# menonsamir/spiral

Measured on AMD Instinct MI355X. Metric: server ms/query + DB GB/s vs HBM roofline, 2^20 x 256B, lower is better.
Workload: dtype u32 residues, 32x32->64-bit integer MAC (two 28-bit CRT primes)

## Files before the change

spiral_amd/csrc/kernels.h:

```cpp
#pragma once
#include <hip/hip_runtime.h>
#include <stdint.h>
#include <stdlib.h>
#include "common.h"

namespace spiral {

struct IndexMap {
    uint32_t inner, outer_stride, off;
    __host__ __device__ uint32_t operator()(uint32_t b) const { return (b / inner) * outer_stride + (b % inner) + off; }
};
inline IndexMap identity_map() { return IndexMap{1u, 1u, 0u}; }

#ifdef SPIRAL_TUNING
inline const char* tuning_env(const char* name) { return getenv(name); }
#else
inline const char* tuning_env(const char*) { return nullptr; }
#endif
struct Options {
    int fold_pair = 1, fold_chain = 1, fwd2 = -1;
    uint32_t fold_blocks = 768, sweep_mfma_min = 2, fwd2_min = 8192;
    size_t db_stage_bytes = (size_t)64 << 20;
    int one_image = 1;
    uint32_t pack_item_group = 0;
};
Options& options();

#ifndef SPIRAL_MAX_LANES
#define SPIRAL_MAX_LANES 8
#endif
constexpr uint32_t kMaxLanes = SPIRAL_MAX_LANES;
struct Lanes {
    uint32_t n = 1;
    int64_t off[kMaxLanes] = {};
#ifdef __HIPCC__
    __device__ __forceinline__ int64_t here() const {
        const uint32_t z = blockIdx.z;
        int64_t o = 0;
#pragma unroll
        for (uint32_t q = 1; q < kMaxLanes; q++) o = z == q ? off[q] : o;
        return o;
    }
    __device__ __forceinline__ int64_t at(int64_t stride) const { return (int64_t)blockIdx.z * stride; }
#endif
};
#ifdef __HIPCC__
template <class T>
__device__ __forceinline__ void lane_shift(T*& p, int64_t words) {
    if (p) p = reinterpret_cast<T*>(reinterpret_cast<uintptr_t>(p) + (intptr_t)words * 8);
}
#endif
struct NoLanes {
    uint32_t n = 1;
#ifdef __HIPCC__
    __device__ __forceinline__ int64_t here() const { return 0; }
    __device__ __forceinline__ int64_t at(int64_t) const { return 0; }
#endif
};
struct Slots {
    uint32_t n = 1;
    int64_t stride = 0;
#ifdef __HIPCC__
    __device__ __forceinline__ int64_t here() const { return (int64_t)blockIdx.z * stride; }
    __device__ __forceinline__ int64_t at(int64_t s) const { return (int64_t)blockIdx.z * s; }
#endif
};
template <class P>
inline typename P::NoLanesT no_lanes(const P& p) {
    typename P::NoLanesT q{};
    static_cast<typename P::Core&>(q) = static_cast<const typename P::Core&>(p);
    return q;
}

struct DeviceTables {
    uint4* fwd = nullptr;
    uint4* inv = nullptr;
    uint64_t* neg1 = nullptr;
    uint64_t* neg1s = nullptr;
};
int tables_get(int device, DeviceTables* out);
void tables_host_rows(uint64_t* out8x2048);

constexpr bool lazy_ok(uint32_t terms) { return (unsigned __int128)terms * (2ull * kP - 1ull) * (kP - 1ull) < ((unsigned __int128)1 << 64); }
static_assert(lazy_ok(56) && lazy_ok(2 * 56) && lazy_ok(128) && !lazy_ok(129), "u64 accumulators hold up to 128 lazy products");

enum FwdLoad : uint32_t {
    LD_RAW = 0,
    LD_DIGIT = 1,
    LD_SDIGIT = 2,
    LD_LIMBS = 3,
    LD_DBGEN = 4,
    LD_PDIGIT = 6,
    LD_DBGEN1 = 7,
    LD_SDIFF = 8,
    LD_PDIFF = 9,
    LD_EXPAND = 5,
    LD_WIRE = 10,
};
constexpr uint32_t kWireCoeffBytes = 7;
constexpr uint32_t kWirePolyBytes = kWireCoeffBytes * 2048u;
enum FwdStore : uint32_t {
    ST_PK = 0,
    ST_REF = 1,
    ST_DB = 2,
    ST_DB1 = 3,
};
enum PackMap : uint32_t {
    PM_GSW = 0,
    PM_FOLD = 1,
    PM_PACK = 2,
};
struct FwdParamsCore {
    const uint64_t* src;
    uint64_t* dst;
    IndexMap src_map;
    IndexMap dst_map;
    uint32_t n_digits;
    uint32_t inv_n_digits, inv_te, inv_to;
    uint32_t bits;
    uint32_t ell;
    uint32_t tinv;
    uint32_t lazy_out;
    uint32_t fold_np;
    uint32_t pmode, pk_num_per;
    uint32_t trial;
    uint64_t total_n;
    uint32_t cnt_e, t_e, t_o;
    const uint8_t* items;
    uint32_t coeff_bits;
    uint64_t items_first;
    uint32_t* err;
    uint64_t seed, p_db;
    uint64_t item_base;
    uint32_t num_per, dim0_shard, j0;
};
template <class L>
struct FwdParamsT : FwdParamsCore {
    using Core = FwdParamsCore;
    using NoLanesT = FwdParamsT<NoLanes>;
    L lanes;
};
using FwdParams = FwdParamsT<Lanes>;
void launch_ntt_forward(const DeviceTables& t, const FwdParams& p, uint32_t load, uint32_t store, uint32_t nblocks, hipStream_t s);

struct ExpandActive {
    uint32_t e_off, o_stride_m1, o_off;
    __host__ __device__ uint32_t index(uint32_t a, uint32_t cnt_e) const {
        return a < cnt_e ? 2u * (a + e_off) : 2u * ((a - cnt_e) * (o_stride_m1 + 1u) + o_off) + 1u;
    }
};

enum InvStore : uint32_t {
    IST_CRT = 0,
    IST_LIMBS = 1,
};
struct InvParamsCore {
    const uint64_t* src;
    uint64_t* dst;
    IndexMap src_map, dst_map;
    uint32_t pre_reduce;
    uint32_t src_ref;
    uint32_t split;
    IndexMap src_map2;
    uint64_t* cv;
    const uint64_t* neg1;
    const uint64_t* neg1s;
    uint32_t num_in, cnt_e;
    ExpandActive act;
    uint32_t auto_t;
    uint32_t create_here;
    const uint64_t* query;
};
template <class L>
struct InvParamsT : InvParamsCore {
    using Core = InvParamsCore;
    using NoLanesT = InvParamsT<NoLanes>;
    L lanes;
// ... 200 lines not shown
```

spiral_amd/csrc/server.cpp:

```cpp
#include <atomic>

#include "db_image.h"
#include "message.h"

using namespace spiral;

thread_local std::string spiral::host::g_err;
using namespace spiral::host;

static std::atomic<uint64_t> g_captures{0};

spiral::Options& spiral::options() {
    static Options o = [] {
        Options v;
        if (const char* e = getenv("SPIRAL_FOLD_PAIR")) v.fold_pair = atoi(e) != 0;
        if (const char* e = getenv("SPIRAL_SWEEP_MFMA")) v.sweep_mfma_min = (uint32_t)strtoul(e, nullptr, 10);
        if (const char* e = getenv("SPIRAL_DB_STAGE_BYTES")) v.db_stage_bytes = (size_t)strtoull(e, nullptr, 10);
        return v;
    }();
    return o;
}

enum GraphId : int {
    G_PRE = 0,
// ... 187 lines not shown

int srv_join_side(spiral_gpu_server* S) {
    if (S->side_pending) {
        HIP_OK(hipStreamWaitEvent(S->stream, S->ev_join, 0));
        S->side_pending = false;
    }
    return 0;
}

enum LaneNeeds : uint32_t {
    NEED_QUERY = 1,
    NEED_DB = 2,
    NEED_RECORDS = 4,
    SHARDED = 8,
    NO_CAPTURE = 16,
    SWEEP_ONLY = 32,
    SHARD_LANES = SHARDED | NO_CAPTURE,
};

int check_lanes(spiral_gpu_server* const* servers, uint32_t n, const char* what, uint32_t needs, Lanes* lanes) {
    if (!servers || n == 0) return fail("%s: no servers", what);
    if (n > kMaxLanes) return fail("%s: at most %u clients per batch", what, kMaxLanes);
    for (uint32_t b = 0; b < n; b++)
        if (!servers[b]) return fail("%s: null server %u", what, b);
    spiral_gpu_server* S = servers[0];
    HIP_OK(hipSetDevice(S->device));
    const bool whole = !(needs & SWEEP_ONLY), sharded = needs & SHARDED;
    lanes->n = n;
    for (uint32_t b = 0; b < n; b++) {
        spiral_gpu_server* L = servers[b];
        if (whole && (((needs & NEED_QUERY) && !L->have_query) || !L->have_pp)) return fail("%s: server %u needs its query and public parameters set first", what, b);
        if ((needs & NEED_DB) && !L->img->loaded) return fail("%s: server %u has no database", what, b);
        if ((needs & NEED_RECORDS) && !L->have_records) return fail("%s: server %u has not converted its query (run_pre first)", what, b);
        if (L->device != S->device || L->dim0_shard != S->dim0_shard || L->s.num_per != S->s.num_per ||
            (whole && (memcmp(&L->p, &S->p, sizeof(S->p)) != 0 || L->j0 != S->j0 || L->j1 != S->j1 || L->cv.words != S->cv.words)))
            return fail("%s: server %u differs from server 0 in parameters, device or shard", what, b);
        if (L->img != S->img) return fail("%s: server %u does not sweep server 0's database image (create_lane / share_db)", what, b);
        if ((sharded || !whole) && L->fold_g_log != S->fold_g_log)
            return fail("%s: server %u has %u fold ranks, server 0 has %u", what, b, 1u << L->fold_g_log, 1u << S->fold_g_log);
        if (sharded && (L->ex_shard.g_log != S->ex_shard.g_log || L->ex_shard.rank != S->ex_shard.rank))
            return fail("%s: server %u has another expansion shard than server 0", what, b);
        if (whole && !sharded && (L->acc != L->acc_own.p || L->fold_g_log || L->ex_shard.g_log))
            return fail("%s: server %u has an external accumulator, fold ranks or a sharded expansion set", what, b);
        if (L->sweep_k_log || (whole && (L->keep_cts || L->overlap || L->side_pending || L->fold_pair != S->fold_pair || L->fold_chain != S->fold_chain)))
            return fail("%s: server %u has keep_cts, a split or staged schedule or other fold options set", what, b);
        for (uint32_t c = 0; c < b; c++)
            if (servers[c] == L) return fail("%s: server %u listed twice", what, b);
        hipStreamCaptureStatus cs = hipStreamCaptureStatusNone;
        if (needs & NO_CAPTURE) HIP_OK(hipStreamIsCapturing(L->stream, &cs));
        if (cs != hipStreamCaptureStatusNone) return fail("%s: server %u's stream is capturing (call it outside stream capture)", what, b);
        lanes->off[b] = L->w_left.p - S->w_left.p;
    }
    return 0;
}

int lanes_join(spiral_gpu_server* const* servers, uint32_t n) {
    spiral_gpu_server* S = servers[0];
    for (uint32_t b = 1; b < n; b++) {
        if (servers[b]->stream == S->stream) continue;
        HIP_OK(hipEventRecord(servers[b]->ev_batch, servers[b]->stream));
        HIP_OK(hipStreamWaitEvent(S->stream, servers[b]->ev_batch, 0));
    }
    return 0;
}
int lanes_release(spiral_gpu_server* const* servers, uint32_t n) {
    spiral_gpu_server* S = servers[0];
    bool other = false;
    for (uint32_t b = 1; b < n; b++) other |= servers[b]->stream != S->stream;
    if (other) HIP_OK(hipEventRecord(S->ev_batch, S->stream));
    for (uint32_t b = 1; b < n; b++)
        if (servers[b]->stream != S->stream) HIP_OK(hipStreamWaitEvent(servers[b]->stream, S->ev_batch, 0));
    return 0;
}

void mark_raw_stale(spiral_gpu_server* const* servers, uint32_t n) {
    for (uint32_t b = 0; b < n; b++) servers[b]->raw_from_acc = false;
}
void mark_swept(spiral_gpu_server* const* servers, uint32_t n) {
    for (uint32_t b = 0; b < n; b++) servers[b]->have_records = true;
    mark_raw_stale(servers, n);
}

void server_records(spiral_gpu_server* const* servers, uint32_t n, const uint32_t** qs, uint64_t** acc) {
    for (uint32_t b = 0; b < n; b++) {
        qs[b] = (const uint32_t*)servers[b]->qs.p;
        acc[b] = servers[b]->acc;
    }
}

int take_pub_params(spiral_gpu_server* S, Form form, const MessageIn& in, const char* what) {
    if (!S) return fail("null server");
    HIP_OK(hipSetDevice(S->device));
    const MessageLayout m = pub_params_layout(S->p, S->s);
    if (form == FORM_NTT && check_ntt_parts(m, in, what)) return -1;
    uint64_t* const dst[kMessageParts] = {S->w_left.p, S->w_right.p, S->w.p, S->v.p};
    S->have_pp = false;
    if (ingest(form, IngestOn{S->stage, S->wire_in, S->tb, S->stream}, m, dst, in, what)) return -1;
    S->have_pp = true;
    return 0;
}
int take_query(spiral_gpu_server* S, Form form, const MessageIn& in, const char* what) {
    if (!S) return fail("null server");
    HIP_OK(hipSetDevice(S->device));
    const MessageLayout m = query_layout(S->p, S->s);
    if (form == FORM_NTT && check_ntt_parts(m, in, what)) return -1;
    uint64_t* const dst[kMessageParts] = {S->query.p};
    S->have_query = S->have_records = false;
    if (ingest(form, IngestOn{S->stage, S->wire_in, S->tb, S->stream}, m, dst, in, what)) return -1;
    S->have_query = true;
    return 0;
}
size_t base_message_bytes(const spiral_gpu_params* p, MessageLayout (*layout)(const spiral_gpu_params&, const spiral_gpu_shape&), Form form) {
    spiral_gpu_shape s;
    return shape_of(p, &s) ? 0 : message_bytes(layout(*p, s), form);
}

int download_pk_as_ref(spiral_gpu_server* S, const uint64_t* pk, IndexMap map, uint64_t* host, size_t npolys) {
    if (npolys == 0) return 0;
    const size_t chunk = 4096;
    if (S->stage.words < std::min(npolys, chunk) * kRefNtt) {
        S->stage.release();
        if (S->stage.alloc(std::min(npolys, chunk) * kRefNtt)) return -1;
    }
    for (size_t done = 0; done < npolys; done += chunk) {
        const size_t n = std::min(chunk, npolys - done);
        IndexMap m = map;
        m.off += (uint32_t)(done / map.inner) * map.outer_stride;
        launch_pk_to_ref(pk, S->stage.p, (uint32_t)n, m, S->stream);
        HIP_OK(hipMemcpyAsync(host + done * kRefNtt, S->stage.p, n * kRefNtt * sizeof(uint64_t), hipMemcpyDeviceToHost, S->stream));
        HIP_OK(hipStreamSynchronize(S->stream));
    }
    return 0;
}

}

extern "C" {

int spiral_gpu_abi_version(void) { return SPIRAL_GPU_ABI_VERSION; }

int spiral_gpu_set_option(const char* name, int64_t value) {
    if (!name) return fail("null option name");
    Options& o = options();
    const std::string n = name;
    if (n == "fold_pair") o.fold_pair = value != 0;
    else if (n == "fold_chain") o.fold_chain = value != 0;
    else if (n == "fold_blocks" && value >= 0) o.fold_blocks = (uint32_t)value;
    else if (n == "sweep_mfma_min" && value >= 0) o.sweep_mfma_min = (uint32_t)value;
    else if (n == "one_image") o.one_image = value != 0;
    else if (n == "fwd2" && value >= -1 && value <= 1) o.fwd2 = (int)value;
    else if (n == "fwd2_min" && value >= 0) o.fwd2_min = (uint32_t)value;
    else if (n == "db_stage_bytes" && value > 0) o.db_stage_bytes = (size_t)value;
    else if (n == "pack_item_group" && value >= 0 && value <= 0xFFFFFFFFll) o.pack_item_group = (uint32_t)value;
    else return fail("unknown option '%s' or value %lld out of range", name, (long long)value);
    return 0;
}
int spiral_gpu_get_option(const char* name, int64_t* value) {
    if (!name || !value) return fail("null argument");
    const Options& o = options();
    const std::string n = name;
    if (n == "fold_pair") *value = o.fold_pair;
    else if (n == "fold_chain") *value = o.fold_chain;
    else if (n == "fold_blocks") *value = o.fold_blocks;
    else if (n == "sweep_mfma_min") *value = o.sweep_mfma_min;
    else if (n == "one_image") *value = o.one_image;
    else if (n == "fwd2") *value = o.fwd2;
    else if (n == "fwd2_min") *value = o.fwd2_min;
    else if (n == "db_stage_bytes") *value = (int64_t)o.db_stage_bytes;
    else if (n == "pack_item_group") *value = o.pack_item_group;
    else if (n == "graph_captures") *value = (int64_t)g_captures.load();
    else return fail("unknown option '%s'", name);
    return 0;
}
const char* spiral_gpu_last_error(void) { return g_err.c_str(); }
int spiral_gpu_device_count(void) {
    int n = 0;
    if (hipGetDeviceCount(&n) != hipSuccess) return 0;
    return n;
}
int spiral_gpu_get_shape(const spiral_gpu_params* p, spiral_gpu_shape* out) { return shape_of(p, out); }
int spiral_gpu_get_tables(uint64_t* out) {
    if (!out) return fail("null argument");
    tables_host_rows(out);
    return 0;
}

int spiral_gpu_ntt_forward(uint64_t* operand, size_t npolys) {
    DeviceTables tb;
    if (current_tables(&tb)) return -1;
    Scratch sc;
    uint64_t* d = sc.upload(operand, npolys * kRefNtt);
    if (!d) return fail("device allocation/upload failed");
    FwdParams fp{};
    fp.src = d;
    fp.dst = d;
    fp.src_map = fp.dst_map = identity_map();
    fp.n_digits = 1;
    launch_ntt_forward(tb, fp, LD_LIMBS, ST_REF, (uint32_t)npolys, 0);
    HIP_OK(hipMemcpy(operand, d, npolys * kRefNtt * sizeof(uint64_t), hipMemcpyDeviceToHost));
    return 0;
}

int spiral_gpu_ntt_inverse(uint64_t* operand, size_t npolys) {
    DeviceTables tb;
    if (current_tables(&tb)) return -1;
    Scratch sc;
    uint64_t* d = sc.upload(operand, npolys * kRefNtt);
    if (!d) return fail("device allocation/upload failed");
    InvParams ip{};
    ip.src = d;
    ip.dst = d;
    ip.src_map = ip.dst_map = identity_map();
    ip.src_ref = 1;
    ip.pre_reduce = 1;
    launch_ntt_inverse(tb, ip, IST_LIMBS, (uint32_t)npolys, 0);
    HIP_OK(hipMemcpy(operand, d, npolys * kRefNtt * sizeof(uint64_t), hipMemcpyDeviceToHost));
    return 0;
}

int spiral_gpu_to_ntt(uint64_t* out, const uint64_t* in, size_t npolys, int reduce) {
    DeviceTables tb;
    if (current_tables(&tb)) return -1;
    Scratch sc;
    uint64_t* d_in = sc.upload(in, npolys * kN);
    uint64_t* d_out = sc.get(npolys * kRefNtt);
    if (!d_in || !d_out) return fail("device allocation/upload failed");
    FwdParams fp{};
    fp.src = d_in;
    fp.dst = d_out;
    fp.src_map = fp.dst_map = identity_map();
    fp.n_digits = 1;
    if (reduce) {
        launch_ntt_forward(tb, fp, LD_RAW, ST_REF, (uint32_t)npolys, 0);
    } else {
        uint64_t* d_pk = sc.get(npolys * kN);
        if (!d_pk) return fail("device allocation failed");
        fp.dst = d_pk;
        fp.bits = 32;
        launch_ntt_forward(tb, fp, LD_DIGIT, ST_PK, (uint32_t)npolys, 0);
        launch_pk_to_ref(d_pk, d_out, (uint32_t)npolys, identity_map(), 0);
    }
    HIP_OK(hipMemcpy(out, d_out, npolys * kRefNtt * sizeof(uint64_t), hipMemcpyDeviceToHost));
    return 0;
}

int spiral_gpu_from_ntt(uint64_t* out, const uint64_t* in, size_t npolys) {
    DeviceTables tb;
    if (current_tables(&tb)) return -1;
    Scratch sc;
    uint64_t* d_in = sc.upload(in, npolys * kRefNtt);
    uint64_t* d_out = sc.get(npolys * kN);
    if (!d_in || !d_out) return fail("device allocation/upload failed");
    InvParams ip{};
    ip.src = d_in;
    ip.dst = d_out;
    ip.src_map = ip.dst_map = identity_map();
    ip.src_ref = 1;
    ip.pre_reduce = 1;
    launch_ntt_inverse(tb, ip, IST_CRT, (uint32_t)npolys, 0);
    HIP_OK(hipMemcpy(out, d_out, npolys * kN * sizeof(uint64_t), hipMemcpyDeviceToHost));
    return 0;
}


int spiral_gpu_time_ntt(size_t npolys, int iters, float* fwd_ms, float* inv_ms) {
    if (!fwd_ms || !inv_ms || iters <= 0 || npolys == 0) return fail("bad argument");
    DeviceTables tb;
    if (current_tables(&tb)) return -1;
    Scratch sc;
    uint64_t* d_raw = sc.get(npolys * kN);
    uint64_t* d_pk = sc.get(npolys * kN);
    if (!d_raw || !d_pk) return fail("device allocation failed");
    HIP_OK(hipMemset(d_raw, 0x5a, npolys * kN * sizeof(uint64_t)));
    hipEvent_t e[3];
    for (auto& x : e) HIP_OK(hipEventCreate(&x));
    FwdParams fp{};
    fp.src = d_raw;
    fp.dst = d_pk;
    fp.src_map = fp.dst_map = identity_map();
    fp.n_digits = 1;
    InvParams ip{};
    ip.src = d_pk;
    ip.dst = d_raw;
    ip.src_map = ip.dst_map = identity_map();
    launch_ntt_forward(tb, fp, LD_RAW, ST_PK, (uint32_t)npolys, 0);
    launch_ntt_inverse(tb, ip, IST_CRT, (uint32_t)npolys, 0);
    HIP_OK(hipEventRecord(e[0], 0));
    for (int i = 0; i < iters; i++) launch_ntt_forward(tb, fp, LD_RAW, ST_PK, (uint32_t)npolys, 0);
    HIP_OK(hipEventRecord(e[1], 0));
    for (int i = 0; i < iters; i++) launch_ntt_inverse(tb, ip, IST_CRT, (uint32_t)npolys, 0);
    HIP_OK(hipEventRecord(e[2], 0));
    HIP_OK(hipEventSynchronize(e[2]));
    HIP_OK(hipEventElapsedTime(fwd_ms, e[0], e[1]));
    HIP_OK(hipEventElapsedTime(inv_ms, e[1], e[2]));
    *fwd_ms /= iters;
    *inv_ms /= iters;
    for (auto& x : e) (void)hipEventDestroy(x);
    return 0;
}

int spiral_gpu_time_ntt_digits(size_t npolys, uint32_t n_digits, int iters, float* ms) {
    if (!ms || iters <= 0 || npolys == 0 || n_digits < 1 || n_digits > 56) return fail("bad argument");
    DeviceTables tb;
    if (current_tables(&tb)) return -1;
    Scratch sc;
    uint64_t* d_raw = sc.get(npolys * kN);
    uint64_t* d_pk = sc.get(npolys * n_digits * kN);
    if (!d_raw || !d_pk) return fail("device allocation failed");
    HIP_OK(hipMemset(d_raw, 0x5a, npolys * kN * sizeof(uint64_t)));
    hipEvent_t e[2];
    for (auto& x : e) HIP_OK(hipEventCreate(&x));
    FwdParams fp{};
    fp.src = d_raw;
    fp.dst = d_pk;
    fp.src_map = fp.dst_map = identity_map();
    fp.n_digits = n_digits;
    fp.bits = get_bits_per(n_digits);
    launch_ntt_forward(tb, fp, LD_DIGIT, ST_PK, (uint32_t)(npolys * n_digits), 0);
    HIP_OK(hipEventRecord(e[0], 0));
    for (int i = 0; i < iters; i++) launch_ntt_forward(tb, fp, LD_DIGIT, ST_PK, (uint32_t)(npolys * n_digits), 0);
    HIP_OK(hipEventRecord(e[1], 0));
    HIP_OK(hipEventSynchronize(e[1]));
// ... 1774 lines not shown
```

spiral_amd/csrc/sweep.hip:

```cpp
#include <cstdlib>
#include "common.h"
#include "kernels.h"

namespace spiral {

typedef unsigned long long u64x2 __attribute__((ext_vector_type(2)));

__device__ __forceinline__ void mac6(uint64_t (&a)[6], uint32_t p0, uint32_t p1, uint32_t p2, uint32_t b0, uint32_t b1, uint32_t b2, uint64_t w) {
    const uint32_t bl = lo32(w), bh = hi32(w);
    a[0] += (uint64_t)p0 * bl;
    a[1] += (uint64_t)p1 * bl;
    a[2] += (uint64_t)p2 * bl;
    a[3] += (uint64_t)b0 * bh;
    a[4] += (uint64_t)b1 * bh;
    a[5] += (uint64_t)b2 * bh;
}
__device__ __forceinline__ void mac_j(uint64_t (&a)[6], const uint4* q, uint64_t w0, uint64_t w1) {
    const uint4 qa = q[0], qb = q[1], qc = q[2];
    mac6(a, qa.x, qa.y, qa.z, qa.w, qb.x, qb.y, w0);
    mac6(a, qb.z, qb.w, qc.x, qc.y, qc.z, qc.w, w1);
}
__device__ __forceinline__ void reduce6(uint64_t (&a)[6]) {
#pragma unroll
    for (int r = 0; r < 3; r++) {
        a[r] = mod_p(a[r]);
        a[3 + r] = mod_b(a[3 + r]);
    }
}
__device__ __forceinline__ void store_acc(uint64_t* acc, const uint64_t (&a)[6], uint32_t ic, uint32_t z, uint32_t g_log, uint32_t ls_log) {
    const uint32_t i0 = ic >> 1, c = ic & 1u;
    const uint32_t ii = acc_pos(i0, g_log, ls_log);
#pragma unroll
    for (uint32_t r = 0; r < 3; r++) acc[((size_t)(6u * ii + 2u * r + c)) * kN + z] = pack((uint32_t)a[r], (uint32_t)a[3 + r]);
}

#ifndef SPIRAL_SWEEP_Z
#define SPIRAL_SWEEP_Z 16
#endif
constexpr uint32_t kSweepZ = SPIRAL_SWEEP_Z;
constexpr uint32_t kSweepRow = 64 * 3 + 1;
typedef unsigned int u32x4 __attribute__((ext_vector_type(4)));

template <int JJ>
__device__ __forceinline__ void mac_packed_j(uint64_t (&a)[6], const uint4* q, const uint32_t (&d)[28]) {
    const uint4 qa = q[0], qb = q[1], qc = q[2];
    const uint32_t p0 = field28<4 * JJ>(d), b0 = field28<4 * JJ + 1>(d), p1 = field28<4 * JJ + 2>(d), b1 = field28<4 * JJ + 3>(d);
    a[0] += (uint64_t)qa.x * p0;
    a[1] += (uint64_t)qa.y * p0;
    a[2] += (uint64_t)qa.z * p0;
    a[3] += (uint64_t)qa.w * b0;
    a[4] += (uint64_t)qb.x * b0;
    a[5] += (uint64_t)qb.y * b0;
    a[0] += (uint64_t)qb.z * p1;
    a[1] += (uint64_t)qb.w * p1;
    a[2] += (uint64_t)qc.x * p1;
    a[3] += (uint64_t)qc.y * b1;
    a[4] += (uint64_t)qc.z * b1;
    a[5] += (uint64_t)qc.w * b1;
}
constexpr uint32_t kQStage = 8 * 24;
struct SweepBatch {
    const uint32_t* qs[kSweepMaxBatch];
    uint64_t* acc[kSweepMaxBatch];
};
template <int MODE, int NB = 1, uint32_t Z = kSweepZ, bool GS = false>
__global__ __launch_bounds__(Z * 64) void sweep_kernel(const uint64_t* __restrict__ db, SweepBatch bt, uint32_t nic, uint32_t dim0, uint32_t g_log, uint32_t ls_log,
                                                             uint32_t icb0, uint32_t n_icb, uint32_t g_extra) {
    static_assert(NB == 1 || MODE == 0, "batched sweeps use the wide geometry");
    const uint32_t* __restrict__ qs = bt.qs[0];
    uint64_t* __restrict__ acc = bt.acc[0];
    constexpr bool WIDE = MODE == 0;
    constexpr uint32_t kShWords = MODE == 2 ? (Z * kQStage * 2 > Z * kSweepRow ? Z * kQStage * 2 : Z * kSweepRow) : Z * kSweepRow;
    __shared__ __attribute__((aligned(16))) uint64_t sh[kShWords];
    const uint32_t lane = threadIdx.x & 63u, wv = __builtin_amdgcn_readfirstlane(threadIdx.x >> 6);
    const uint32_t w = WIDE ? 64u : nic, pz = 64u / w, nblk = nic / w;
    uint32_t work = blockIdx.x;
    if ((gridDim.x & 7u) == 0) work = (blockIdx.x & 7u) * (gridDim.x >> 3) + (blockIdx.x >> 3);
    const uint32_t zg = work / n_icb, icb = icb0 + (work - zg * n_icb);
    const uint32_t groups = dim0 >> 3;
    const uint32_t ztile = WIDE ? zg * Z + wv : zg, tile = ztile * nblk + icb;
    const uint32_t gper = WIDE ? groups : (groups + Z - 1u) / Z;
    const uint32_t gfirst = WIDE ? 0u : min(wv * gper, groups), glast = WIDE ? groups : min(gfirst + gper, groups);
    const uint32_t z = WIDE ? ztile : ztile * pz + lane / w;
    const u32x4* dbp = reinterpret_cast<const u32x4*>(db) + (size_t)tile * groups * 7u * 64u + lane;
    const uint4* q = reinterpret_cast<const uint4*>(qs) + (size_t)z * dim0 * 3u;
    uint64_t a[6] = {0, 0, 0, 0, 0, 0};
    uint64_t ax[NB > 1 ? NB - 1 : 1][6] = {};
    for (uint32_t g0 = gfirst; g0 < glast; g0 += 16) {
        const uint32_t gend = min(g0 + 16u, glast);
#pragma unroll 2
        for (uint32_t g = g0; g < gend; g++) {
            uint32_t d[28];
#pragma unroll
            for (uint32_t k = 0; k < 7; k++) {
                const u32x4 v = __builtin_nontemporal_load(dbp + ((size_t)g * 7u + k) * 64u);
                d[4 * k] = v.x;
                d[4 * k + 1] = v.y;
                d[4 * k + 2] = v.z;
                d[4 * k + 3] = v.w;
            }
            const uint4* qg = q + (size_t)g * 24u;
            if constexpr (MODE == 2) {
                uint4* qst = reinterpret_cast<uint4*>(sh) + wv * kQStage;
                const uint4* qsrc = reinterpret_cast<const uint4*>(qs);
                __builtin_amdgcn_fence(__ATOMIC_ACQ_REL, "wavefront");
                __builtin_amdgcn_wave_barrier();
                for (uint32_t t = lane; t < pz * 24u; t += 64u) {
                    const uint32_t zi = t / 24u, off = t - zi * 24u;
                    qst[t] = qsrc[((size_t)(ztile * pz + zi) * dim0 + (size_t)g * 8u) * 3u + off];
                }
                __builtin_amdgcn_fence(__ATOMIC_ACQ_REL, "wavefront");
                __builtin_amdgcn_wave_barrier();
                qg = qst + (lane / w) * 24u;
            }
            mac_packed_j<0>(a, qg, d);
            mac_packed_j<1>(a, qg + 3, d);
            mac_packed_j<2>(a, qg + 6, d);
            mac_packed_j<3>(a, qg + 9, d);
            mac_packed_j<4>(a, qg + 12, d);
            mac_packed_j<5>(a, qg + 15, d);
            mac_packed_j<6>(a, qg + 18, d);
            mac_packed_j<7>(a, qg + 21, d);
            if constexpr (NB > 1) {
#pragma unroll
                for (int b = 1; b < NB; b++) {
                    const uint4* qb = reinterpret_cast<const uint4*>(bt.qs[b]) + (size_t)z * dim0 * 3u + (size_t)g * 24u;
                    mac_packed_j<0>(ax[b - 1], qb, d);
                    mac_packed_j<1>(ax[b - 1], qb + 3, d);
                    mac_packed_j<2>(ax[b - 1], qb + 6, d);
                    mac_packed_j<3>(ax[b - 1], qb + 9, d);
                    mac_packed_j<4>(ax[b - 1], qb + 12, d);
                    mac_packed_j<5>(ax[b - 1], qb + 15, d);
                    mac_packed_j<6>(ax[b - 1], qb + 18, d);
                    mac_packed_j<7>(ax[b - 1], qb + 21, d);
                }
            }
        }
        reduce6(a);
        if constexpr (NB > 1) {
#pragma unroll
            for (int b = 1; b < NB; b++) reduce6(ax[b - 1]);
        }
    }
    if constexpr (MODE == 2) __syncthreads();
#pragma unroll
    for (int b = 0; b < NB; b++) {
    if constexpr (NB > 1) {
        if (b > 0) {
            __syncthreads();
            acc = bt.acc[b];
#pragma unroll
            for (int r = 0; r < 6; r++) a[r] = ax[b - 1][r];
        }
    }
#pragma unroll
    for (uint32_t r = 0; r < 3; r++) sh[wv * kSweepRow + lane * 3u + r] = pack((uint32_t)a[r], (uint32_t)a[3 + r]);
    __syncthreads();
    if constexpr (WIDE) {
#pragma unroll
        for (uint32_t m = 0; m < 3; m++) {
            const uint32_t idx = threadIdx.x + Z * 64u * m, res = idx / Z, zz = idx - res * Z;
            const uint32_t col = res / 3u, r = res - col * 3u, ic = icb * 64u + col, i0 = ic >> 1, c = ic & 1u;
            uint32_t ii = acc_pos(i0, g_log, ls_log);
            if constexpr (GS) ii += (i0 & ((1u << g_log) - 1u)) * g_extra;
            acc[((size_t)(6u * ii + 2u * r + c)) * kN + zg * Z + zz] = sh[zz * kSweepRow + res];
        }
    } else if (threadIdx.x < 192u) {
        const uint32_t sl = threadIdx.x / 3u, r = threadIdx.x - sl * 3u, zz = sl / w, col = sl - zz * w, i0 = col >> 1, c = col & 1u;
        uint64_t sp = 0, sb = 0;
#pragma unroll
        for (uint32_t v = 0; v < Z; v++) {
            const uint64_t x = sh[v * kSweepRow + threadIdx.x];
            sp += lo32(x);
            sb += hi32(x);
        }
        uint32_t ii = acc_pos(i0, g_log, ls_log);
        if constexpr (GS) ii += (i0 & ((1u << g_log) - 1u)) * g_extra;
        acc[((size_t)(6u * ii + 2u * r + c)) * kN + zg * pz + zz] = pack(mod_p(sp), mod_b(sb));
    }
    }
}

__global__ __launch_bounds__(256) void sweep_small_kernel(const uint64_t* __restrict__ db, const uint32_t* __restrict__ qs,
                                                          uint64_t* __restrict__ acc, uint32_t nic, uint32_t dim0, uint32_t g_log, uint32_t ls_log) {
    const uint32_t g = blockIdx.x * 256u + threadIdx.x;
    const uint32_t z = g / nic, ic = g - z * nic;
    if (z >= kN) return;
    const uint4* q = reinterpret_cast<const uint4*>(qs) + (size_t)z * dim0 * 3u;
    uint64_t a[6] = {0, 0, 0, 0, 0, 0};
    for (uint32_t j = 0; j < dim0; j++) {
        const ulonglong2 w = *reinterpret_cast<const ulonglong2*>(db + db_word_index(z, j, ic, 0, nic, dim0));
        mac_j(a, q + j * 3u, w.x, w.y);
        if ((j & 127u) == 127u) reduce6(a);
    }
    reduce6(a);
    store_acc(acc, a, ic, z, g_log, ls_log);
}

static uint32_t log2u(uint32_t x) {
    uint32_t l = 0;
    while ((1u << l) < x) l++;
    return l;
}
bool sweep_batch_ok(uint32_t num_per, uint32_t jm_total) { return 2 * num_per >= 64 && db_packed(2 * num_per, jm_total / 2); }
void launch_sweep_batch(const uint64_t* db, const uint32_t* const* qs, uint64_t* const* acc, uint32_t n, uint32_t num_per, uint32_t jm_total, uint32_t g_log,
                        hipStream_t s, uint32_t g_extra) {
    const uint32_t nic = 2 * num_per, dim0 = jm_total / 2, ls_log = log2u(num_per) - g_log;
    SweepBatch bt{};
    for (uint32_t b = 0; b < n; b++) {
        bt.qs[b] = qs[b];
        bt.acc[b] = acc[b];
    }
    const dim3 grid((kN / kSweepZ) * (nic >> 6)), block(kSweepZ * 64);
    switch (n) {
        case 2:
            if (g_extra)
                hipLaunchKernelGGL((sweep_kernel<0, 2, kSweepZ, true>), grid, block, 0, s, db, bt, nic, dim0, g_log, ls_log, 0u, nic >> 6, g_extra);
            else
                hipLaunchKernelGGL((sweep_kernel<0, 2>), grid, block, 0, s, db, bt, nic, dim0, g_log, ls_log, 0u, nic >> 6, 0u);
            break;
        default: abort();
    }
}
bool sweep_stages_ok(uint32_t num_per, uint32_t jm_total, uint32_t g_log, uint32_t k_log) {
    if (k_log == 0) return true;
    const uint32_t nic = 2 * num_per;
    return (num_per & (num_per - 1)) == 0 && db_packed(nic, jm_total / 2) && (nic >> 6) >= (1u << k_log) && log2u(num_per) >= g_log + k_log;
}
void launch_sweep(const uint64_t* db, const uint32_t* qs, uint64_t* acc, uint32_t num_per, uint32_t jm_total, uint32_t g_log, hipStream_t s, uint32_t k_log,
                  int stage) {
    const uint32_t nic = 2 * num_per, dim0 = jm_total / 2;
    if (dim0 == 0) return;
    const uint32_t ls_log = log2u(num_per) - g_log - k_log;
    SweepBatch bt{};
    bt.qs[0] = qs;
    bt.acc[0] = acc;
    if (db_packed(nic, dim0)) {
        static const bool stage_recs = [] {
            const char* e = tuning_env("SPIRAL_SWEEP_STAGE");
            return e ? atoi(e) != 0 : true;
        }();
        if (nic >= 64) {
            const uint32_t nblk = nic >> 6, per = nblk >> k_log;
            const uint32_t icb0 = stage < 0 ? 0u : (uint32_t)stage * per, n_icb = stage < 0 ? nblk : per;
            if ((kN / kSweepZ) * n_icb < 256u)
                hipLaunchKernelGGL((sweep_kernel<0, 1, 8>), dim3((kN / 8) * n_icb), dim3(8 * 64), 0, s, db, bt, nic, dim0, g_log, ls_log, icb0, n_icb, 0u);
            else
                hipLaunchKernelGGL(sweep_kernel<0>, dim3((kN / kSweepZ) * n_icb), dim3(kSweepZ * 64), 0, s, db, bt, nic, dim0, g_log, ls_log, icb0, n_icb, 0u);
        } else if (nic >= 8 && stage_recs)
            hipLaunchKernelGGL(sweep_kernel<2>, dim3(kN / (64 / nic)), dim3(kSweepZ * 64), 0, s, db, bt, nic, dim0, g_log, ls_log, 0u, 1u, 0u);
        else
            hipLaunchKernelGGL(sweep_kernel<1>, dim3(kN / (64 / nic)), dim3(kSweepZ * 64), 0, s, db, bt, nic, dim0, g_log, ls_log, 0u, 1u, 0u);
    } else {
        const uint32_t threads = kN * nic;
        hipLaunchKernelGGL(sweep_small_kernel, dim3((threads + 255) / 256), dim3(256), 0, s, db, qs, acc, nic, dim0, g_log, ls_log);
    }
}

__global__ __launch_bounds__(256) void db_relayout_kernel(const uint64_t* __restrict__ ref, uint64_t* __restrict__ dev, uint32_t num_per, uint32_t dim0,
                                                          uint32_t j0, uint32_t dim0_shard, uint32_t z0, uint32_t nz) {
    const uint32_t nic = 2 * num_per;
    const size_t o = (size_t)blockIdx.x * 256u + threadIdx.x;
    const size_t per_z = (size_t)dim0_shard * nic * 2u;
    const uint32_t zl = (uint32_t)(o / per_z);
    if (zl >= nz) return;
    size_t rem = o - (size_t)zl * per_z;
    const uint32_t m = (uint32_t)(rem & 1u);
    rem >>= 1;
    const uint32_t ic = (uint32_t)(rem % nic), jl = (uint32_t)(rem / nic);
    const uint32_t ii = ic >> 1, c = ic & 1u, j = j0 + jl;
    const uint64_t v = ref[(size_t)zl * ((size_t)num_per * 2u * dim0 * 2u) + (size_t)ii * (2u * dim0 * 2u) + (size_t)c * (dim0 * 2u) + (size_t)j * 2u + m];
    db_put_word(dev, pk_pos(z0 + zl), jl, ic, m, nic, dim0_shard, pack(lo32(v) % kP, hi32(v) % kB));
}
void launch_db_relayout(const uint64_t* db_ref, uint64_t* db_dev, uint32_t num_per, uint32_t dim0, uint32_t j0, uint32_t dim0_shard, uint32_t z0,
                        uint32_t nz, hipStream_t s) {
    const size_t words = (size_t)nz * dim0_shard * 2u * num_per * 2u;
    hipLaunchKernelGGL(db_relayout_kernel, dim3((uint32_t)((words + 255) / 256)), dim3(256), 0, s, db_ref, db_dev, num_per, dim0, j0, dim0_shard, z0, nz);
}

__global__ __launch_bounds__(256) void db_read_item_kernel(const uint64_t* __restrict__ dev, uint64_t* __restrict__ out, uint32_t num_per, uint32_t dim0_shard,
                                                           uint32_t jl, uint32_t ii, uint32_t limbs) {
    const uint32_t z = blockIdx.x * 256u + threadIdx.x, mc = blockIdx.y, m = mc >> 1, c = mc & 1u;
    const uint64_t v = limbs ? db_get_word_limbs(dev, pk_pos(z), jl, ii * 2u + c, m, 2u * num_per, dim0_shard)
                             : db_get_word(dev, pk_pos(z), jl, ii * 2u + c, m, 2u * num_per, dim0_shard);
    out[(size_t)mc * (2 * kN) + z] = lo32(v);
    out[(size_t)mc * (2 * kN) + kN + z] = hi32(v);
}
void launch_db_read_item(const uint64_t* db_dev, uint64_t* out_ref, uint32_t num_per, uint32_t dim0_shard, uint32_t j_local, uint32_t ii, hipStream_t s,
                         bool limbs) {
    hipLaunchKernelGGL(db_read_item_kernel, dim3(kN / 256, 4), dim3(256), 0, s, db_dev, out_ref, num_per, dim0_shard, j_local, ii, limbs ? 1u : 0u);
}
__global__ __launch_bounds__(256) void db_read_slots_kernel(const uint64_t* __restrict__ dev, uint64_t* __restrict__ out, uint32_t num_per, uint32_t dim0_shard,
                                                            uint32_t z0, uint32_t nz, uint32_t ii0, uint32_t n_ii, uint32_t limbs) {
    const size_t o = (size_t)blockIdx.x * 256u + threadIdx.x, per_z = (size_t)n_ii * 2u * dim0_shard * 2u;
    const uint32_t zl = (uint32_t)(o / per_z);
    if (zl >= nz) return;
    size_t rem = o - (size_t)zl * per_z;
    const uint32_t m = (uint32_t)(rem & 1u);
    rem >>= 1;
    const uint32_t jl = (uint32_t)(rem % dim0_shard);
    rem /= dim0_shard;
    const uint32_t c = (uint32_t)(rem & 1u), ii = ii0 + (uint32_t)(rem >> 1);
    out[o] = limbs ? db_get_word_limbs(dev, pk_pos(z0 + zl), jl, ii * 2u + c, m, 2u * num_per, dim0_shard)
                   : db_get_word(dev, pk_pos(z0 + zl), jl, ii * 2u + c, m, 2u * num_per, dim0_shard);
}
void launch_db_read_slots(const uint64_t* db_dev, uint64_t* out, uint32_t num_per, uint32_t dim0_shard, uint32_t z0, uint32_t nz, uint32_t ii0, uint32_t n_ii,
                          hipStream_t s, bool limbs) {
    const size_t words = (size_t)nz * n_ii * 2u * dim0_shard * 2u;
    hipLaunchKernelGGL(db_read_slots_kernel, dim3((uint32_t)((words + 255) / 256)), dim3(256), 0, s, db_dev, out, num_per, dim0_shard, z0, nz, ii0, n_ii,
                       limbs ? 1u : 0u);
}

__global__ __launch_bounds__(256) void qs_from_reoriented_kernel(const uint64_t* __restrict__ re, uint32_t* __restrict__ qs, uint32_t jm_total) {
    const size_t g = (size_t)blockIdx.x * 256u + threadIdx.x;
    if (g >= (size_t)kN * jm_total) return;
    const uint64_t* src = re + g * 4u;
    const uint32_t z = (uint32_t)(g / jm_total), jm = (uint32_t)(g - (size_t)z * jm_total);
    uint32_t* rec = qs + ((size_t)pk_pos(z) * jm_total + jm) * 6u;
#pragma unroll
    for (uint32_t r = 0; r < 3; r++) {
        rec[r] = lo32(src[r]) % kP;
        rec[3 + r] = hi32(src[r]) % kB;
    }
}
void launch_qs_from_reoriented(const uint64_t* reoriented, uint32_t* qs, uint32_t jm_total, hipStream_t s) {
    const size_t n = (size_t)kN * jm_total;
    hipLaunchKernelGGL(qs_from_reoriented_kernel, dim3((uint32_t)((n + 255) / 256)), dim3(256), 0, s, reoriented, qs, jm_total);
}

__global__ __launch_bounds__(256) void fill_db_random_kernel(uint64_t* db, uint32_t nic, uint32_t dim0, uint64_t seed) {
    const uint64_t nwords = (uint64_t)kN * dim0 * nic * 2u, stride = (uint64_t)gridDim.x * 256u;
    for (uint64_t i = (uint64_t)blockIdx.x * 256u + threadIdx.x; i < nwords; i += stride) {
        uint64_t x = seed + i + 0x9E3779B97F4A7C15ull;
        x = (x ^ (x >> 30)) * 0xBF58476D1CE4E5B9ull;
        x = (x ^ (x >> 27)) * 0x94D049BB133111EBull;
        x ^= x >> 31;
        const uint32_t m = (uint32_t)(i & 1u), ic = (uint32_t)((i >> 1) % nic);
        const uint64_t rest = (i >> 1) / nic;
        const uint32_t j = (uint32_t)(rest % dim0), z = (uint32_t)(rest / dim0);
        db_put_word(db, z, j, ic, m, nic, dim0, pack((uint32_t)(x & 0xffffffffull) % kP, (uint32_t)(x >> 32) % kB));
    }
}
void launch_fill_db_random(uint64_t* db_dev, uint32_t num_per, uint32_t dim0_shard, uint64_t seed, hipStream_t s) {
    hipLaunchKernelGGL(fill_db_random_kernel, dim3(4096), dim3(256), 0, s, db_dev, 2 * num_per, dim0_shard, seed);
}

}
```

Before: 0.7379.

## Replace one-shot sweep grid with persistent per-CU item loop and register prefetch

Replaces the per-tile sweep kernel launch with a persistent kernel sized to the CU count. Each block walks a strided list of (z-group, column-block) items, with an XCD-aware split of the work. DB groups are prefetched two steps ahead into registers using nontemporal loads, and query records are read through a constant address-space pointer. Results go through a double-buffered shared-memory transpose to the accumulator. The intent is to hide HBM latency and cut block launch and scheduling overhead, at the cost of more register pressure and more complex control flow.

```diff
diff --git a/spiral_amd/csrc/kernels.h b/spiral_amd/csrc/kernels.h
--- a/spiral_amd/csrc/kernels.h
+++ b/spiral_amd/csrc/kernels.h
@@ -23,6 +23,7 @@
     size_t db_stage_bytes = (size_t)64 << 20;
     int one_image = 1;
     uint32_t pack_item_group = 0;
+    uint32_t sweep_groups = 0;
 };
 Options& options();
 
diff --git a/spiral_amd/csrc/server.cpp b/spiral_amd/csrc/server.cpp
--- a/spiral_amd/csrc/server.cpp
+++ b/spiral_amd/csrc/server.cpp
@@ -363,6 +363,7 @@
     else if (n == "fwd2_min" && value >= 0) o.fwd2_min = (uint32_t)value;
     else if (n == "db_stage_bytes" && value > 0) o.db_stage_bytes = (size_t)value;
     else if (n == "pack_item_group" && value >= 0 && value <= 0xFFFFFFFFll) o.pack_item_group = (uint32_t)value;
+    else if (n == "sweep_groups" && value >= 0 && value <= 0xFFFFll) o.sweep_groups = (uint32_t)value;
     else return fail("unknown option '%s' or value %lld out of range", name, (long long)value);
     return 0;
 }
@@ -379,6 +380,7 @@
     else if (n == "fwd2_min") *value = o.fwd2_min;
     else if (n == "db_stage_bytes") *value = (int64_t)o.db_stage_bytes;
     else if (n == "pack_item_group") *value = o.pack_item_group;
+    else if (n == "sweep_groups") *value = o.sweep_groups;
     else if (n == "graph_captures") *value = (int64_t)g_captures.load();
     else return fail("unknown option '%s'", name);
     return 0;
diff --git a/spiral_amd/csrc/sweep.hip b/spiral_amd/csrc/sweep.hip
--- a/spiral_amd/csrc/sweep.hip
+++ b/spiral_amd/csrc/sweep.hip
@@ -1,3 +1,5 @@
+#include <algorithm>
+#include <atomic>
 #include <cstdlib>
 #include "common.h"
 #include "kernels.h"
@@ -44,6 +46,24 @@
 template <int JJ>
 __device__ __forceinline__ void mac_packed_j(uint64_t (&a)[6], const uint4* q, const uint32_t (&d)[28]) {
     const uint4 qa = q[0], qb = q[1], qc = q[2];
+    const uint32_t p0 = field28<4 * JJ>(d), b0 = field28<4 * JJ + 1>(d), p1 = field28<4 * JJ + 2>(d), b1 = field28<4 * JJ + 3>(d);
+    a[0] += (uint64_t)qa.x * p0;
+    a[1] += (uint64_t)qa.y * p0;
+    a[2] += (uint64_t)qa.z * p0;
+    a[3] += (uint64_t)qa.w * b0;
+    a[4] += (uint64_t)qb.x * b0;
+    a[5] += (uint64_t)qb.y * b0;
+    a[0] += (uint64_t)qb.z * p1;
+    a[1] += (uint64_t)qb.w * p1;
+    a[2] += (uint64_t)qc.x * p1;
+    a[3] += (uint64_t)qc.y * b1;
+    a[4] += (uint64_t)qc.z * b1;
+    a[5] += (uint64_t)qc.w * b1;
+}
+typedef const __attribute__((address_space(4))) u32x4* rec_ptr;
+template <int JJ>
+__device__ __forceinline__ void mac_packed_j(uint64_t (&a)[6], rec_ptr q, const uint32_t (&d)[28]) {
+    const u32x4 qa = q[0], qb = q[1], qc = q[2];
     const uint32_t p0 = field28<4 * JJ>(d), b0 = field28<4 * JJ + 1>(d), p1 = field28<4 * JJ + 2>(d), b1 = field28<4 * JJ + 3>(d);
     a[0] += (uint64_t)qa.x * p0;
     a[1] += (uint64_t)qa.y * p0;
@@ -181,6 +201,102 @@
     }
 }
 
+constexpr uint32_t kSweepAhead = 2;
+template <uint32_t Z>
+__global__ __launch_bounds__(Z * 64) void sweep_items_kernel(const uint64_t* __restrict__ db, const uint32_t* __restrict__ qs, uint64_t* __restrict__ acc, uint32_t nic,
+                                                                   uint32_t dim0, uint32_t g_log, uint32_t ls_log, uint32_t icb0, uint32_t n_icb) {
+    __shared__ __attribute__((aligned(16))) uint64_t sh[2][Z * kSweepRow];
+    const uint32_t lane = threadIdx.x & 63u, wv = __builtin_amdgcn_readfirstlane(threadIdx.x >> 6);
+    const uint32_t nblk = nic >> 6, groups = dim0 >> 3;
+    const bool by_xcd = (gridDim.x & 7u) == 0;
+    const uint32_t n_items = (kN / Z) * n_icb, step = by_xcd ? gridDim.x >> 3 : gridDim.x, span = by_xcd ? n_items >> 3 : n_items;
+    const uint32_t slot = by_xcd ? blockIdx.x >> 3 : blockIdx.x, first = (by_xcd ? (blockIdx.x & 7u) * span : 0u) + slot;
+    if (slot >= span) return;
+    const uint32_t n_mine = (span - slot + step - 1u) / step, trips = n_mine * groups;
+    const u32x4* dbv = reinterpret_cast<const u32x4*>(db);
+    const rec_ptr qv = (rec_ptr) reinterpret_cast<uintptr_t>(qs);
+    const size_t tile_words = (size_t)groups * 7u * 64u;
+    auto tile_of = [&](uint32_t work, uint32_t& zg, uint32_t& icb) {
+        zg = work / n_icb;
+        icb = icb0 + (work - zg * n_icb);
+        return (zg * Z + wv) * nblk + icb;
+    };
+    uint32_t zg, icb;
+    uint32_t lk = 0, lg = 0;
+    const u32x4* lrow = dbv + (size_t)tile_of(first, zg, icb) * tile_words;
+    uint32_t d[kSweepAhead][28];
+    auto next_group = [&]() {
+        const bool more = lk < n_mine;
+        const u32x4* p = lrow + (size_t)lg * (7u * 64u) + (more ? lane : 0u);
+        if (more && ++lg == groups) {
+            if (++lk < n_mine) {
+                uint32_t z_, i_;
+                lg = 0;
+                lrow = dbv + (size_t)tile_of(first + lk * step, z_, i_) * tile_words;
+            } else
+                lg = groups - 1u;
+        }
+        return p;
+    };
+    auto load_group = [&](uint32_t (&dd)[28], const u32x4* p) {
+#pragma unroll
+        for (uint32_t k = 0; k < 7; k++) {
+            const u32x4 v = __builtin_nontemporal_load(p + k * 64u);
+            dd[4 * k] = v.x;
+            dd[4 * k + 1] = v.y;
+            dd[4 * k + 2] = v.z;
+            dd[4 * k + 3] = v.w;
+        }
+    };
+#pragma unroll
+    for (uint32_t s = 0; s < kSweepAhead; s++) load_group(d[s], next_group());
+    uint32_t ck = 0, cg = 0, buf = 0;
+    rec_ptr q = qv + (size_t)(zg * Z + wv) * dim0 * 3u;
+    uint64_t a[6] = {0, 0, 0, 0, 0, 0};
+    for (uint32_t t = 0; t < trips; t += kSweepAhead) {
+#pragma unroll
+        for (uint32_t s = 0; s < kSweepAhead; s++) {
+            const u32x4* ahead = next_group();
+            const rec_ptr qg = q + (size_t)cg * 24u;
+            mac_packed_j<0>(a, qg, d[s]);
+            mac_packed_j<1>(a, qg + 3, d[s]);
+            mac_packed_j<2>(a, qg + 6, d[s]);
+            mac_packed_j<3>(a, qg + 9, d[s]);
+            mac_packed_j<4>(a, qg + 12, d[s]);
+            mac_packed_j<5>(a, qg + 15, d[s]);
+            mac_packed_j<6>(a, qg + 18, d[s]);
+            mac_packed_j<7>(a, qg + 21, d[s]);
+            __builtin_amdgcn_sched_barrier(0);
+            load_group(d[s], ahead);
+            if (t + s < trips) {
+                cg++;
+                if ((cg & 15u) == 0 || cg == groups) reduce6(a);
+                if (cg == groups) {
+                    uint64_t* row = sh[buf];
+#pragma unroll
+                    for (uint32_t r = 0; r < 3; r++) row[wv * kSweepRow + lane * 3u + r] = pack((uint32_t)a[r], (uint32_t)a[3 + r]);
+                    __syncthreads();
+#pragma unroll
+                    for (uint32_t m = 0; m < 3; m++) {
+                        const uint32_t idx = threadIdx.x + Z * 64u * m, res = idx / Z, zz = idx - res * Z;
+                        const uint32_t col = res / 3u, r = res - col * 3u, ic = icb * 64u + col, i0 = ic >> 1, c = ic & 1u;
+                        const uint32_t ii = acc_pos(i0, g_log, ls_log);
+                        acc[((size_t)(6u * ii + 2u * r + c)) * kN + zg * Z + zz] = row[zz * kSweepRow + res];
+                    }
+                    buf ^= 1u;
+#pragma unroll
+                    for (int r = 0; r < 6; r++) a[r] = 0;
+                    cg = 0;
+                    if (++ck < n_mine) {
+                        tile_of(first + ck * step, zg, icb);
+                        q = qv + (size_t)(zg * Z + wv) * dim0 * 3u;
+                    }
+                }
+            }
+        }
+    }
+}
+
 __global__ __launch_bounds__(256) void sweep_small_kernel(const uint64_t* __restrict__ db, const uint32_t* __restrict__ qs,
                                                           uint64_t* __restrict__ acc, uint32_t nic, uint32_t dim0, uint32_t g_log, uint32_t ls_log) {
     const uint32_t g = blockIdx.x * 256u + threadIdx.x;
@@ -201,6 +317,18 @@
     uint32_t l = 0;
     while ((1u << l) < x) l++;
     return l;
+}
+static uint32_t device_cus() {
+    static std::atomic<uint32_t> cus[64];
+    int dev = 0;
+    if (hipGetDevice(&dev) != hipSuccess || dev < 0 || dev >= 64) return 256u;
+    uint32_t n = cus[dev].load(std::memory_order_relaxed);
+    if (n == 0) {
+        int v = 0;
+        n = hipDeviceGetAttribute(&v, hipDeviceAttributeMultiprocessorCount, dev) == hipSuccess && v > 0 ? (uint32_t)v : 256u;
+        cus[dev].store(n, std::memory_order_relaxed);
+    }
+    return n;
 }
 bool sweep_batch_ok(uint32_t num_per, uint32_t jm_total) { return 2 * num_per >= 64 && db_packed(2 * num_per, jm_total / 2); }
 void launch_sweep_batch(const uint64_t* db, const uint32_t* const* qs, uint64_t* const* acc, uint32_t n, uint32_t num_per, uint32_t jm_total, uint32_t g_log,
@@ -243,10 +371,12 @@
         if (nic >= 64) {
             const uint32_t nblk = nic >> 6, per = nblk >> k_log;
             const uint32_t icb0 = stage < 0 ? 0u : (uint32_t)stage * per, n_icb = stage < 0 ? nblk : per;
+            const uint32_t want = options().sweep_groups ? options().sweep_groups : device_cus();
             if ((kN / kSweepZ) * n_icb < 256u)
-                hipLaunchKernelGGL((sweep_kernel<0, 1, 8>), dim3((kN / 8) * n_icb), dim3(8 * 64), 0, s, db, bt, nic, dim0, g_log, ls_log, icb0, n_icb, 0u);
+                hipLaunchKernelGGL(sweep_items_kernel<8>, dim3(std::min(want, (kN / 8) * n_icb)), dim3(8 * 64), 0, s, db, qs, acc, nic, dim0, g_log, ls_log, icb0, n_icb);
             else
-                hipLaunchKernelGGL(sweep_kernel<0>, dim3((kN / kSweepZ) * n_icb), dim3(kSweepZ * 64), 0, s, db, bt, nic, dim0, g_log, ls_log, icb0, n_icb, 0u);
+                hipLaunchKernelGGL(sweep_items_kernel<kSweepZ>, dim3(std::min(want, (kN / kSweepZ) * n_icb)), dim3(kSweepZ * 64), 0, s, db, qs, acc, nic, dim0, g_log,
+                                   ls_log, icb0, n_icb);
         } else if (nic >= 8 && stage_recs)
             hipLaunchKernelGGL(sweep_kernel<2>, dim3(kN / (64 / nic)), dim3(kSweepZ * 64), 0, s, db, bt, nic, dim0, g_log, ls_log, 0u, 1u, 0u);
         else
```

Result: no change. 0.7405 (+0.4%).
